# dwcoen1234/longfellow-zk

Hardware: AMD Instinct MI355X
Metric: FFT field-elems/s (batched FFT 2^20 x 1024 rows, Fp128) (higher is better)
Workload: dtype u128 (Fp128 Montgomery, 4 x u32 limbs); 1 GPU; batched FFT 2^20 points x 1024 rows per GPU, Fp128 fftb, in place in HBM; field=Fp128 p=2^128-2^108+1, rows_per_gpu=1024, n=1048576, parallelism=rows sharded x1

## Files before the change

longfellow-zk_amd/csrc/fft.hip:

```cpp
#include <string>
#include <type_traits>

#include "ctx.h"
#include "fp_tile_arith.h"

int lf_lch14_fft_bitsliced(lfgpu_ctx* c, int k, int inverse, size_t rows, unsigned l, u64 coset, void* d_B, size_t ld);

#define TILE_ELTS 8192u

struct TilePlan {
  const elt_t* src;
  elt_t* dst;
  long long src_row, dst_row;
  long long src_tile, dst_tile;
  long long sk, sc, dk, dc;
  u32 logT, logC, nbatch;
  u32 kfast_src, kfast_dst;
  u32 wlds;
};

__device__ __forceinline__ u32 bitrev(u32 x, u32 bits) { return bits ? (__brev(x) >> (32 - bits)) : 0; }

__device__ __forceinline__ u32 lds_slot(u32 k, u32 c, u32 logT, u32 logC) {
  u32 slot = (k << logC) + c;
// ... 102 lines not shown
      if (R == 3) fp_radix_round<O, 3, FFT_THREADS>(s, W, wsh, p.logT, p.logC, st, tid);
      else if (R == 2) fp_radix_round<O, 2, FFT_THREADS>(s, W, wsh, p.logT, p.logC, st, tid);
      else fp_radix_round<O, 1, FFT_THREADS>(s, W, wsh, p.logT, p.logC, st, tid);
    }
    __syncthreads();
    st += R;
  }
  for (u32 e = tid; e < T * C; e += FFT_THREADS) {
    u32 j, c;
    if (p.kfast_dst) { j = e & (T - 1); c = e >> p.logT; } else { c = e & (C - 1); j = e >> p.logC; }
    if (cbase + c >= p.nbatch) continue;
    elt_t v = ld16(&s[lds_slot(j, c, p.logT, p.logC)]);
    if (tw_lo) {
      const u32 col = cbase + c, ex = j * col;
      if (ex) {
        if (tw_hi) {
          elt_t t = ld16(&tw_lo[ex & 1023]);
          if (ex >> 10) t = O::mul_tw(t, ld16(&tw_hi[ex >> 10]));
          v = O::mul_tw(v, t);
        } else {
          v = O::mul_tw(v, ld16(&tw_lo[(size_t)j * p.nbatch + col]));
        }
      }
    }
    st16(dst + (long long)j * p.dk + (long long)c * p.dc, v);
  }
}

template <class O>
struct T4Ops : O {
  static __device__ __forceinline__ elt_t add_lazy(elt_t a, elt_t b) { return O::add(a, b); }
  static __device__ __forceinline__ elt_t canon(elt_t a) { return a; }
  static __device__ __forceinline__ elt_t mul_tw_sw(elt_t a, elt_t w) { return O::mul_tw(a, w); }
};
#if defined(__HIP_DEVICE_COMPILE__)
template <>
struct T4Ops<Fp128Ops> : Fp128Ops {
  static __device__ __forceinline__ elt_t add(elt_t a, elt_t b) { return fpt_add(a, b); }
  static __device__ __forceinline__ elt_t add_lazy(elt_t a, elt_t b) { return fpt_add_lazy(a, b); }
  static __device__ __forceinline__ elt_t canon(elt_t a) { return fpt_canon(a); }
  static __device__ __forceinline__ elt_t sub(elt_t a, elt_t b) { return fpt_sub(a, b); }
  static __device__ __forceinline__ elt_t mul_tw(elt_t a, elt_t w) { return fpt_mul(a, w); }
  static __device__ __forceinline__ elt_t mul_tw_sw(elt_t a, elt_t w) { return fpt_mul_sw(a, w); }
};
#endif

__device__ __forceinline__ u32 t4_slot(u32 p, u32 c, u32 p7) { return ((p << 2) | c) ^ p7; }
__device__ __forceinline__ u32 t4_wslot(u32 i) { return i ^ ((i >> 4) & 15u); }

enum : u32 { T4_CANON = 0, T4_LAZY = 1, T4_LAZY_OUT = 2 };
template <class O, u32 ST, u32 R, bool ROUND0, u32 LZ = T4_CANON>
__device__ __forceinline__ void t4_stages(elt_t* x, u32 j, const elt_t* wl, const elt_t* __restrict__ W, u32 wshift) {
#pragma unroll
  for (u32 t = 0; t < R; ++t) {
    const u32 half = 1u << t;
#pragma unroll
    for (u32 a = 0; a < (1u << R); ++a) {
      if (a & half) continue;
      const u32 jj = j + (a & (half - 1)) * (1u << ST), sh = 9 - ST - t;
      if (!ROUND0) x[a + half] = T4Ops<O>::mul_tw(x[a + half], ld16(&wl[t4_wslot(jj << sh)]));
      else if (a & (half - 1)) x[a + half] = T4Ops<O>::mul_tw(x[a + half], ld16(&W[(size_t)(jj << sh) << wshift]));
      const bool last = LZ == T4_LAZY_OUT && t == R - 1;
      const bool full = LZ == T4_CANON || last || (ROUND0 && ((t == 0 && a != 0) || (t == 1 && a == 4)));
      const elt_t u = last ? T4Ops<O>::canon(x[a]) : x[a], v = x[a + half];
      x[a] = full ? T4Ops<O>::add(u, v) : T4Ops<O>::add_lazy(u, v);
      x[a + half] = T4Ops<O>::sub(u, v);
    }
  }
}

template <class O, u32 LZ>
__device__ __forceinline__ void t4_round0(elt_t* s, const elt_t* y, u32 kb, u32 c, const elt_t* wl, const elt_t* __restrict__ W, u32 wshift) {
  elt_t x[8];
#pragma unroll
  for (u32 a = 0; a < 8; ++a) x[a] = y[((a & 1) << 2) | (a & 2) | (a >> 2)];
  t4_stages<O, 0, 3, true, LZ>(x, 0, wl, W, wshift);
  const u32 b = __brev(kb) >> 25, s0 = t4_slot(8 * b, c, b >> 4), s1 = t4_slot(8 * b + 1, c, b >> 4);
#pragma unroll
// ... 223 lines not shown
  fp_fft_tile_1024x4_tws_body<O, KFAST_SRC, true>(p, W, wshift, tw, row_fast);
}
template <class O, bool KFAST_SRC>
__global__ __launch_bounds__(512, 4) void fp_fft_tile_1024x4_tws_canon(TilePlan p, const elt_t* __restrict__ W, u32 wshift,
                                                                       const elt_t* __restrict__ tw, u32 row_fast) {
  fp_fft_tile_1024x4_tws_body<O, KFAST_SRC, false>(p, W, wshift, tw, row_fast);
}

__device__ __forceinline__ u32 t4w_swz(u32 p) { return (p >> 7) ^ ((p >> 4) & 12u); }
__device__ __forceinline__ u32 t4w_slot(u32 p, u32 c) { return ((p << 2) | c) ^ t4w_swz(p); }

template <u32 ST>
__device__ __forceinline__ u32 t4w_tw_index(u32 j, u32 m) {
  const u32 t = m < 1 ? 0 : m < 3 ? 1 : 2, k = m + 1 - (1u << t);
  return (j + (k << ST)) << (9 - ST - t);
}
enum : u32 { T4W_R0 = 0, T4W_R1 = 1, T4W_R1_J0 = 2 };
template <class O, u32 MODE>
__device__ __forceinline__ void t4w_stages(elt_t* x, const elt_t* w) {
#pragma unroll
  for (u32 t = 0; t < 3; ++t) {
    const u32 half = 1u << t;
#pragma unroll
    for (u32 a = 0; a < 8; ++a) {
      if (a & half) continue;
      const u32 k = a & (half - 1);
      const bool skip = MODE != T4W_R1 && k == 0, full = MODE == T4W_R0 && ((t == 0 && a != 0) || (t == 1 && a == 4));
      const elt_t u = x[a], v = !skip ? T4Ops<O>::mul_tw_sw(x[a + half], w[half - 1 + k]) : MODE == T4W_R1_J0 ? T4Ops<O>::canon(x[a + half]) : x[a + half];
      x[a] = full ? T4Ops<O>::add(u, v) : T4Ops<O>::add_lazy(u, v);
      x[a + half] = T4Ops<O>::sub(u, v);
    }
  }
}
template <class O>
__device__ __forceinline__ void t4w_round0(elt_t* s, const elt_t* y, u32 kb, u32 c, const elt_t* w) {
  elt_t x[8];
#pragma unroll
  for (u32 a = 0; a < 8; ++a) x[a] = y[((a & 1) << 2) | (a & 2) | (a >> 2)];
  t4w_stages<O, T4W_R0>(x, w);
  const u32 s0 = t4w_slot((__brev(kb) >> 25) << 3, c);
#pragma unroll
  for (u32 a = 0; a < 8; ++a) st16(&s[(s0 ^ (4 * (a & 3))) + 16 * (a >> 2)], x[a]);
}
template <class O, u32 MODE>
__device__ __forceinline__ void t4w_round1_wave(elt_t* s, u32 s0, const elt_t* w) {
  elt_t x[8];
#pragma unroll
  for (u32 a = 0; a < 8; ++a) x[a] = ld16(&s[s0 + 32 * a]);
  t4w_stages<O, MODE>(x, w);
#pragma unroll
  for (u32 a = 0; a < 8; ++a) st16(&s[s0 + 32 * a], x[a]);
}
template <class O>
__device__ __forceinline__ void t4w_round1(elt_t* s, u32 tid, u32 j, const elt_t* w) {
  const u32 c = tid & 3, h = (tid >> 2) & 15;
  const u32 s0 = t4w_slot(64 * h + j, c);
  if (j == 0) {
    asm volatile("; round 1, j = 0");
    t4w_round1_wave<O, T4W_R1_J0>(s, s0, w);
    asm volatile("; round 1, j = 0: stored");
  } else {
    asm volatile("; round 1, j > 0");
    t4w_round1_wave<O, T4W_R1>(s, s0, w);
    asm volatile("; round 1, j > 0: stored");
  }
}
template <class O>
__device__ __forceinline__ void t4w_round2(elt_t* s, u32 e, const elt_t* wl, const elt_t* __restrict__ W, u32 wshift) {
  const u32 c = e & 3, h = e >> 8, j = (e >> 2) & 63;
  const u32 s0 = t4w_slot(256 * h + j, c);
  elt_t x[4];
#pragma unroll
  for (u32 a = 0; a < 4; ++a) x[a] = ld16(&s[(s0 ^ t4w_swz(64 * a)) + 256 * a]);
  t4_stages<O, 6, 2, false, T4_LAZY>(x, j, wl, W, wshift);
#pragma unroll
  for (u32 a = 0; a < 4; ++a) st16(&s[(s0 ^ t4w_swz(64 * a)) + 256 * a], x[a]);
}
__device__ __forceinline__ void t4w_round3_load(elt_t* x, const elt_t* s, u32 e) {
  const u32 s0 = t4w_slot(e >> 2, e & 3);
#pragma unroll
  for (u32 a = 0; a < 4; ++a) x[a] = ld16(&s[(s0 ^ (2 * a)) + 1024 * a]);
}

template <class O, bool KFAST_SRC>
__global__ __launch_bounds__(512, 4) void fp_fft_tile_1024x4_tw2(TilePlan p, const elt_t* __restrict__ W, u32 wshift,
                                                                 const elt_t* __restrict__ tw, u32 row_fast) {
  extern __shared__ elt_t s[];
  elt_t* const wl = s + 4096;
  const u32 tid = threadIdx.x, j1 = __builtin_amdgcn_readfirstlane(tid >> 6);
  u32 bx, by;
  if (KFAST_SRC) {
    bx = row_fast ? blockIdx.y : blockIdx.x;
    by = row_fast ? blockIdx.x : blockIdx.y;
  } else {
    t4_xcd_order(p.nbatch >> 2, blockIdx.x, bx, by);
  }
  elt_t w0[7] = {}, w1[7];
  {
    const u32 c = KFAST_SRC ? tid >> 7 : tid & 3, kb = KFAST_SRC ? tid & 127 : tid >> 2;
    const elt_t* src = p.src + (long long)by * p.src_row + (long long)bx * p.src_tile;
    const u32 sk = (u32)p.sk, off = kb * sk + c * (u32)p.sc;
    elt_t y[8], t[8];
#pragma unroll
    for (u32 a = 0; a < 8; ++a) y[a] = ld16(src + (off + 128 * a * sk));
    if (KFAST_SRC) {
      const elt_t* twt = tw + ((size_t)bx << 12);
      const u32 toff = (c << 10) + kb;
#pragma unroll
      for (u32 a = 0; a < 8; ++a) t[a] = ld16(twt + (toff + 128 * a));
    }
    const elt_t wv = ld16(&W[(size_t)tid << wshift]);
#pragma unroll
    for (u32 m = 0; m < 7; ++m) {
      w1[m] = ld16(&W[(size_t)t4w_tw_index<3>(j1, m) << wshift]);
      if (m >= 4) w0[m] = ld16(&W[(size_t)t4w_tw_index<0>(0, m) << wshift]);
    }
#pragma unroll
    for (u32 m = 0; m < 7; ++m) {
      asm volatile("" : "+s"(w1[m].lo), "+s"(w1[m].hi));
      if (m >= 4) asm volatile("" : "+s"(w0[m].lo), "+s"(w0[m].hi));
    }
    w0[2] = w0[5];
    __builtin_amdgcn_sched_barrier(0);
    if (KFAST_SRC) {
#pragma unroll
      for (u32 a = 0; a < 8; ++a) y[a] = T4Ops<O>::mul_tw(y[a], t[a]);
    }
    t4w_round0<O>(s, y, kb, c, w0);
    st16(&wl[t4_wslot(tid)], wv);
  }
  __syncthreads();
  t4w_round1<O>(s, tid, j1, w1);
  __syncthreads();
#pragma unroll
  for (u32 g = 0; g < 2; ++g) t4w_round2<O>(s, tid + 512 * g, wl, W, wshift);
  __syncthreads();
  {
    elt_t* dst = p.dst + (long long)by * p.dst_row + (long long)bx * p.dst_tile;
    const u32 dk = (u32)p.dk, dc = (u32)p.dc;
#pragma unroll
    for (u32 g = 0; g < 2; ++g) {
      const u32 e = tid + 512 * g, c = e & 3, j = e >> 2;
      elt_t x[4];
      t4w_round3_load(x, s, e);
      t4_stages<O, 8, 2, false, KFAST_SRC ? T4_LAZY_OUT : T4_LAZY>(x, j, wl, W, wshift);
#pragma unroll
      for (u32 a = 0; a < 4; ++a) st16(dst + ((j + 256 * a) * dk + c * dc), x[a]);
    }
  }
}

struct LchTables {
  const elt_t* tbl;
  const elt_t* base;
  u32 nb;
  u32 off[16];
};

template <int FFT_THREADS>
__global__ __launch_bounds__(FFT_THREADS) void lch_fft_tile(TilePlan p, int inverse, LchTables t) {
  extern __shared__ elt_t s[];
  const u32 T = 1u << p.logT, C = 1u << p.logC, tid = threadIdx.x;
  const u32 cbase = blockIdx.x << p.logC;
  const elt_t* src = p.src + (long long)blockIdx.y * p.src_row + (long long)blockIdx.x * p.src_tile;
  elt_t* dst = p.dst + (long long)blockIdx.y * p.dst_row + (long long)blockIdx.x * p.dst_tile;

  for (u32 e = tid; e < T * C; e += FFT_THREADS) {
    u32 k, c;
    if (p.kfast_src) { k = e & (T - 1); c = e >> p.logT; } else { c = e & (C - 1); k = e >> p.logC; }
    elt_t v = elt_zero();
    if (cbase + c < p.nbatch) v = ld16(src + (long long)k * p.sk + (long long)c * p.sc);
    st16(&s[(k << p.logC) + c], v);
  }
  __syncthreads();
  for (u32 step = 0; step < p.logT; ++step) {
    const u32 ii = inverse ? step : (p.logT - 1 - step);
    const u32 sz = 1u << ii;
    for (u32 e = tid; e < (T >> 1) * C; e += FFT_THREADS) {
// ... 21 lines not shown
    __syncthreads();
  }
  for (u32 e = tid; e < T * C; e += FFT_THREADS) {
    u32 j, c;
    if (p.kfast_dst) { j = e & (T - 1); c = e >> p.logT; } else { c = e & (C - 1); j = e >> p.logC; }
    if (cbase + c >= p.nbatch) continue;
    st16(dst + (long long)j * p.dk + (long long)c * p.dc, ld16(&s[(j << p.logC) + c]));
  }
}

template <class O>
static int set_lds_limit_fp(lfgpu_ctx* c) {
  LF_HIP(c, hipFuncSetAttribute((const void*)fp_fft_tile<O, 1024, true>, hipFuncAttributeMaxDynamicSharedMemorySize, 160 * 1024));
  LF_HIP(c, hipFuncSetAttribute((const void*)fp_fft_tile<O, 1024, false>, hipFuncAttributeMaxDynamicSharedMemorySize, 160 * 1024));
  LF_HIP(c, hipFuncSetAttribute((const void*)fp_fft_tile<O, 512, true>, hipFuncAttributeMaxDynamicSharedMemorySize, 160 * 1024));
  LF_HIP(c, hipFuncSetAttribute((const void*)fp_fft_tile<O, 512, false>, hipFuncAttributeMaxDynamicSharedMemorySize, 160 * 1024));
  return LFGPU_OK;
}
static int set_lds_limit(lfgpu_ctx* c) {
  if (!(c->attr_done & 1u)) {
    if (const char* e = getenv("LFGPU_TILE_LOG")) {
      int v = atoi(e);
      if (v == 12 || v == 13) c->tile_log = v;
    }
    LF_TRY(set_lds_limit_fp<Fp128Ops>(c));
    const void* const t4[] = {(const void*)fp_fft_tile_1024x4<Fp128Ops, false, true>,
                              (const void*)fp_fft_tile_1024x4<Fp128Ops, true, false>,
                              (const void*)fp_fft_tile_1024x4_persist<Fp128Ops>,
                              (const void*)fp_fft_tile_1024x4_tws<Fp128Ops, false>,
                              (const void*)fp_fft_tile_1024x4_tws<Fp128Ops, true>,
                              (const void*)fp_fft_tile_1024x4_tws_canon<Fp128Ops, false>,
                              (const void*)fp_fft_tile_1024x4_tws_canon<Fp128Ops, true>,
                              (const void*)fp_fft_tile_1024x4_tw2<Fp128Ops, false>,
                              (const void*)fp_fft_tile_1024x4_tw2<Fp128Ops, true>};
    for (const void* k : t4) LF_HIP(c, hipFuncSetAttribute(k, hipFuncAttributeMaxDynamicSharedMemorySize, 160 * 1024));
    LF_TRY(set_lds_limit_fp<F64x2Ops<true>>(c));
    LF_TRY(set_lds_limit_fp<F64x2Ops<false>>(c));
    LF_HIP(c, hipFuncSetAttribute((const void*)lch_fft_tile<1024>, hipFuncAttributeMaxDynamicSharedMemorySize, TILE_ELTS * 16));
    LF_HIP(c, hipFuncSetAttribute((const void*)lch_fft_tile<512>, hipFuncAttributeMaxDynamicSharedMemorySize, TILE_ELTS * 16));
    c->attr_done |= 1u;
  }
  return LFGPU_OK;
}

static size_t fp_lds_bytes(TilePlan& p) {
  const size_t tile = ((size_t)16 << p.logT) << p.logC, tw = (size_t)8 << p.logT;
  p.wlds = tile + tw <= 160u * 1024u ? 1u : 0u;
  return p.wlds ? tile + tw : tile;
}
template <class O, class... Args>
static void launch_fp(lfgpu_ctx* c, dim3 grid, size_t lds, const TilePlan& p, Args... args) {
  if (c->tile_log == 13) {
    if (p.wlds) hipLaunchKernelGGL((fp_fft_tile<O, 1024, true>), grid, dim3(1024), lds, c->stream, p, args...);
    else hipLaunchKernelGGL((fp_fft_tile<O, 1024, false>), grid, dim3(1024), lds, c->stream, p, args...);
  } else {
    if (p.wlds) hipLaunchKernelGGL((fp_fft_tile<O, 512, true>), grid, dim3(512), lds, c->stream, p, args...);
    else hipLaunchKernelGGL((fp_fft_tile<O, 512, false>), grid, dim3(512), lds, c->stream, p, args...);
  }
}
struct FpSwitches {
  bool tile1024;
  int persist;
  int twside;
  bool other_plan;
  bool lazy;
  bool r1wave;
  bool two_level;
  bool row_fast;
};
static const FpSwitches& fp_switches() {
  static const FpSwitches sw = [] {
    const auto num = [](const char* name, int dflt) { return getenv(name) ? atoi(getenv(name)) : dflt; };
    FpSwitches w;
    w.tile1024 = num("LFGPU_FP_TILE1024", 1) != 0;
    w.persist = num("LFGPU_FP_PERSIST", 1);
    w.twside = num("LFGPU_FP_TWSIDE", 1);
    w.other_plan = getenv("LFGPU_FP_PERSIST") || getenv("LFGPU_FP_TILE1024");
    w.lazy = num("LFGPU_FP_LAZY", 1) != 0;
    w.r1wave = num("LFGPU_FP_R1WAVE", 1) != 0;
    w.two_level = num("LFGPU_FP_TW", 0) == 2;
    w.row_fast = num("LFGPU_FP_ROWFAST", 1) != 0;
    return w;
  }();
  return sw;
}
static bool tile_1024x4_fits(const TilePlan& p, bool kfast_src, bool offsets32) {
  if (p.logT != 10 || p.logC != 2 || !p.wlds || p.kfast_src != (kfast_src ? 1u : 0u) || p.kfast_dst != 0 || (p.nbatch & 3) != 0) return false;
  return !offsets32 || (p.sk >= 0 && p.sc >= 0 && p.dk >= 0 && p.dc >= 0 && (u64)p.sk * 1024 + (u64)p.sc * 4 <= 0xffffffffu &&
                        (u64)p.dk * 1024 + (u64)p.dc * 4 <= 0xffffffffu);
}
template <class O>
static bool launch_tile_1024x4_persist(lfgpu_ctx* c, u32 rows, size_t lds, const TilePlan& p, const elt_t* W, u32 wshift, const elt_t* tw) {
  const int mode = fp_switches().persist;
  const u32 ncb = p.nbatch >> 2;
  u32 parts = rows;
  if (mode <= 0 || !tile_1024x4_fits(p, false, true)) return false;
  if (mode >= 2) {
    static const int per_cu = [lds] {
      int n = 0;
      if (hipOccupancyMaxActiveBlocksPerMultiprocessor(&n, (const void*)fp_fft_tile_1024x4_persist<O>, 512, lds) != hipSuccess)
        n = 0;
      return n < 1 ? 1 : n;
    }();
    const u32 fill = (u32)per_cu * (u32)c->num_cu;
    parts = fill / ncb;
    if (parts < 1) parts = 1;
    if (parts > rows) parts = rows;
  }
  if ((u64)ncb * parts > 0x7fffffffu) return false;
  const dim3 grid(ncb * parts);
  hipLaunchKernelGGL((fp_fft_tile_1024x4_persist<O>), grid, dim3(512), lds, c->stream, p, W, wshift, tw, rows, parts);
  return true;
}
template <class O, bool KFAST_SRC, bool TW>
static bool launch_tile_1024x4(lfgpu_ctx* c, dim3 grid, size_t lds, const TilePlan& p, const elt_t* W, u32 wshift, const elt_t* tw,
                               u32 row_fast) {
  if constexpr (std::is_same<O, Fp128Ops>::value) {
    if (fp_switches().tile1024 && c->tile_log == 12 && tile_1024x4_fits(p, KFAST_SRC, false)) {
      if constexpr (!KFAST_SRC && TW)
        if (launch_tile_1024x4_persist<O>(c, row_fast ? grid.x : grid.y, lds, p, W, wshift, tw)) return true;
      hipLaunchKernelGGL((fp_fft_tile_1024x4<O, KFAST_SRC, TW>), grid, dim3(512), lds, c->stream, p, W, wshift, tw, row_fast);
      return true;
    }
  }
  return false;
}
template <class O>
static int fp_twside_mode(const lfgpu_ctx* c, u32 logn1, size_t rows, bool two_level) {
  const int mode = fp_switches().other_plan ? 0 : fp_switches().twside;
  if (!std::is_same<O, Fp128Ops>::value || two_level || c->tile_log != 12 || logn1 != 10 || rows > (0x7fffffffu >> 8)) return 0;
  return mode < 0 ? 0 : mode;
}
template <class O, bool KFAST_SRC>
static bool launch_tile_1024x4_tws(lfgpu_ctx* c, u32 rows, size_t lds, const TilePlan& p, const elt_t* W, u32 wshift, const elt_t* tw,
                                   u32 row_fast) {
  if constexpr (std::is_same<O, Fp128Ops>::value) {
    const u32 ncb = p.nbatch >> 2;
    if (!tile_1024x4_fits(p, KFAST_SRC, true) || (u64)ncb * rows > 0x7fffffffu) return false;
    if (KFAST_SRC && (p.sk != 1 || p.sc != 1024 || p.src_tile != 4096)) return false;
    if (KFAST_SRC && (row_fast ? ncb : rows) > 65535) row_fast = !row_fast;
    const dim3 grid = !KFAST_SRC ? dim3(ncb * rows) : row_fast ? dim3(rows, ncb) : dim3(ncb, rows);
    if (!fp_switches().lazy) hipLaunchKernelGGL((fp_fft_tile_1024x4_tws_canon<O, KFAST_SRC>), grid, dim3(512), lds, c->stream, p, W, wshift, tw, row_fast);
    else if (fp_switches().r1wave) hipLaunchKernelGGL((fp_fft_tile_1024x4_tw2<O, KFAST_SRC>), grid, dim3(512), lds, c->stream, p, W, wshift, tw, row_fast);
    else hipLaunchKernelGGL((fp_fft_tile_1024x4_tws<O, KFAST_SRC>), grid, dim3(512), lds, c->stream, p, W, wshift, tw, row_fast);
    return true;
  }
  return false;
}
template <class... Args>
static void launch_lch(lfgpu_ctx* c, dim3 grid, size_t lds, Args... args) {
  if (c->tile_log == 13)
    hipLaunchKernelGGL(lch_fft_tile<1024>, grid, dim3(1024), lds, c->stream, args...);
  else
    hipLaunchKernelGGL(lch_fft_tile<512>, grid, dim3(512), lds, c->stream, args...);
}

template <class O>
static elt_t fp_reroot(elt_t w, u64 n, u64 r) {
  while (r < n) {
    w = O::hmul(w, w);
    r += r;
  }
  return w;
}

static std::string keyf(const char* fmt, ...) {
  char buf[256];
  va_list ap;
  va_start(ap, fmt);
  vsnprintf(buf, sizeof(buf), fmt, ap);
  va_end(ap);
  return std::string(buf);
}

static TilePlan plan_single(const lfgpu_ctx* c, void* A, size_t rows, u32 logn, size_t ld) {
// ... 359 lines not shown
```

longfellow-zk_amd/csrc/fp_tile_arith.h:

```cpp
#pragma once
#include "fields.h"

#if defined(__HIP_DEVICE_COMPILE__)
__device__ __forceinline__ elt_t fpt_add(elt_t a, elt_t b) {
  FP_W(a, a0, a1, a2, a3);
  FP_W(b, b0, b1, b2, b3);
  u32 s0, s1, s2, s3, d0, d1, d2, d3;
  u64 c;
  asm("v_add_co_u32 %0, vcc, %9, %13\n\t"
      "s_nop 1\n\t"
      "v_addc_co_u32 %1, vcc, %10, %14, vcc\n\t"
      "s_nop 1\n\t"
      "v_addc_co_u32 %2, vcc, %11, %15, vcc\n\t"
      "s_nop 1\n\t"
      "v_addc_co_u32 %3, %8, %12, %16, vcc\n\t"
      "v_subrev_co_u32 %4, vcc, 1, %0\n\t"
      "s_nop 1\n\t"
      "v_subbrev_co_u32 %5, vcc, 0, %1, vcc\n\t"
      "s_nop 1\n\t"
      "v_subbrev_co_u32 %6, vcc, 0, %2, vcc\n\t"
      "s_nop 1\n\t"
      "v_subb_co_u32 %7, vcc, %3, %17, vcc\n\t"
      "s_nop 1\n\t"
      "s_andn2_b64 vcc, vcc, %8\n\t"
// ... 139 lines not shown
        "s_nop 1\n\t"
        "v_subb_co_u32 %2, vcc, %15, %6, vcc\n\t"
        "s_nop 1\n\t"
        "v_subb_co_u32 %3, %10, %16, %7, vcc\n\t"
        "v_alignbit_b32 %4, %5, %4, 20\n\t"
        "v_alignbit_b32 %5, %6, %5, 20\n\t"
        "v_alignbit_b32 %6, %7, %6, 20\n\t"
        "v_lshrrev_b32 %7, 20, %7\n\t"
        "v_addc_co_u32 %0, vcc, %0, %4, %9\n\t"
        "s_nop 1\n\t"
        "v_addc_co_u32 %1, vcc, %1, %5, vcc\n\t"
        "s_nop 1\n\t"
        "v_addc_co_u32 %2, vcc, %2, %6, vcc\n\t"
        "s_nop 1\n\t"
        "v_addc_co_u32 %3, %9, %3, %7, vcc\n\t"
        "s_nop 1\n\t"
        "s_andn2_b64 %9, %10, %9\n\t"
        "v_cndmask_b32 %8, 0, %12, %9\n\t"
        "v_addc_co_u32 %0, vcc, 0, %0, %9\n\t"
        "s_nop 1\n\t"
        "v_addc_co_u32 %1, vcc, 0, %1, vcc\n\t"
        "s_nop 1\n\t"
        "v_addc_co_u32 %2, vcc, 0, %2, vcc\n\t"
        "s_nop 1\n\t"
        "v_addc_co_u32 %3, vcc, %8, %3, vcc"
        : "=&v"(d0), "=&v"(d1), "=&v"(d2), "=&v"(d3), "+v"(t0), "+v"(t1), "+v"(t2), "+v"(t3), "=&v"(e3), "=&s"(cy), "=&s"(b)
        : "v"(k), "v"(0xfffff000u), "v"(t4), "v"(t5), "v"(t6), "v"(t7)
        : "vcc", "scc");
  }
  return FP_PACK(d0, d1, d2, d3);
}
__device__ __forceinline__ elt_t fpt_mul(elt_t a, elt_t b) { return fpt_mul_t<false>(a, b); }
__device__ __forceinline__ elt_t fpt_mul_sw(elt_t a, elt_t b) { return fpt_mul_t<true>(a, b); }
#else
LF_HD elt_t fpt_add(elt_t a, elt_t b) { return fp_add_c(a, b); }
LF_HD elt_t fpt_sub(elt_t a, elt_t b) { return fp_sub_c(a, b); }
LF_HD elt_t fpt_canon(elt_t a) { return fp_canon128(a); }
LF_HD elt_t fpt_add_lazy(elt_t a, elt_t b) {
  const u64 lo = a.lo + b.lo, c0 = lo < a.lo, h0 = a.hi + b.hi, hi = h0 + c0;
  if (!((h0 < a.hi) | (hi < c0))) return elt_t{lo, hi};
  return elt_t{lo - FP_P_LO, hi - FP_P_HI - (lo < FP_P_LO)};
}
LF_HD elt_t fpt_mul(elt_t a, elt_t b) { return fp_mul_c(fp_canon128(a), b); }
LF_HD elt_t fpt_mul_sw(elt_t a, elt_t b) { return fpt_mul(a, b); }
#endif
```

Baseline: 48.89 billion field-elems/s.

## Interleave paired Fp128 multiplies and butterflies in inline asm for ILP

```diff
diff --git a/longfellow-zk_amd/csrc/fft.hip b/longfellow-zk_amd/csrc/fft.hip
--- a/longfellow-zk_amd/csrc/fft.hip
+++ b/longfellow-zk_amd/csrc/fft.hip
@@ -158,6 +158,14 @@
   static __device__ __forceinline__ elt_t add_lazy(elt_t a, elt_t b) { return O::add(a, b); }
   static __device__ __forceinline__ elt_t canon(elt_t a) { return a; }
   static __device__ __forceinline__ elt_t mul_tw_sw(elt_t a, elt_t w) { return O::mul_tw(a, w); }
+  static __device__ __forceinline__ void mul2_tw(elt_t& a, elt_t w, elt_t& b, elt_t v) { a = O::mul_tw(a, w), b = O::mul_tw(b, v); }
+  static __device__ __forceinline__ void mul2_tw_sw(elt_t& a, elt_t w, elt_t& b, elt_t v) { mul2_tw(a, w, b, v); }
+  static __device__ __forceinline__ void canon2(elt_t&, elt_t&) {}
+  static __device__ __forceinline__ void bfly_lazy(elt_t& x, elt_t& y) {
+    const elt_t u = x, t = y;
+    x = O::add(u, t), y = O::sub(u, t);
+  }
+  static __device__ __forceinline__ void bfly2_lazy(elt_t& xp, elt_t& yp, elt_t& xq, elt_t& yq) { bfly_lazy(xp, yp), bfly_lazy(xq, yq); }
 };
 #if defined(__HIP_DEVICE_COMPILE__)
 template <>
@@ -168,8 +176,21 @@
   static __device__ __forceinline__ elt_t sub(elt_t a, elt_t b) { return fpt_sub(a, b); }
   static __device__ __forceinline__ elt_t mul_tw(elt_t a, elt_t w) { return fpt_mul(a, w); }
   static __device__ __forceinline__ elt_t mul_tw_sw(elt_t a, elt_t w) { return fpt_mul_sw(a, w); }
+  static __device__ __forceinline__ void mul2_tw(elt_t& a, elt_t w, elt_t& b, elt_t v) { fpt_mul2(a, w, b, v); }
+  static __device__ __forceinline__ void mul2_tw_sw(elt_t& a, elt_t w, elt_t& b, elt_t v) { fpt_mul2_sw(a, w, b, v); }
+  static __device__ __forceinline__ void canon2(elt_t& a, elt_t& b) { fpt_canon2(a, b); }
+  static __device__ __forceinline__ void bfly_lazy(elt_t& x, elt_t& y) { fpt_bfly_lazy(x, y); }
+  static __device__ __forceinline__ void bfly2_lazy(elt_t& xp, elt_t& yp, elt_t& xq, elt_t& yq) { fpt_bfly2_lazy(xp, yp, xq, yq); }
 };
 #endif
+template <class O>
+struct T4Ilp : O {};
+template <class O>
+struct T4IsIlp : std::false_type {};
+template <class O>
+struct T4IsIlp<T4Ilp<O>> : std::true_type {};
+template <class O>
+struct T4Ops<T4Ilp<O>> : T4Ops<O> {};
 
 __device__ __forceinline__ u32 t4_slot(u32 p, u32 c, u32 p7) { return ((p << 2) | c) ^ p7; }
 __device__ __forceinline__ u32 t4_wslot(u32 i) { return i ^ ((i >> 4) & 15u); }
@@ -459,12 +480,79 @@
     }
   }
 }
+struct T4iStage {
+  u32 np, prod[4], nc, can[4], nl, lazy[4], nf, full[4];
+};
+template <u32 MODE>
+constexpr T4iStage t4i_plan(u32 t) {
+  T4iStage s{};
+  const u32 half = 1u << t;
+  for (u32 a = 0; a < 8; ++a) {
+    if (a & half) continue;
+    const bool skip = MODE != T4W_R1 && (a & (half - 1)) == 0, full = MODE == T4W_R0 && ((t == 0 && a != 0) || (t == 1 && a == 4));
+    if (!skip) s.prod[s.np++] = a;
+    else if (MODE == T4W_R1_J0) s.can[s.nc++] = a;
+    if (full) s.full[s.nf++] = a;
+    else s.lazy[s.nl++] = a;
+  }
+  return s;
+}
+template <class O, u32 MODE, u32 T>
+__device__ __forceinline__ void t4i_stage(elt_t* x, const elt_t* w) {
+  constexpr T4iStage S = t4i_plan<MODE>(T);
+  constexpr u32 half = 1u << T, first = half - 1;
+#pragma unroll
+  for (u32 i = 0; i + 1 < S.np; i += 2) {
+    const u32 a = S.prod[i], b = S.prod[i + 1];
+    T4Ops<O>::mul2_tw_sw(x[a + half], w[first + (a & first)], x[b + half], w[first + (b & first)]);
+  }
+  if constexpr (S.np & 1) x[S.prod[S.np - 1] + half] = T4Ops<O>::mul_tw_sw(x[S.prod[S.np - 1] + half], w[first + (S.prod[S.np - 1] & first)]);
+#pragma unroll
+  for (u32 i = 0; i + 1 < S.nc; i += 2) T4Ops<O>::canon2(x[S.can[i] + half], x[S.can[i + 1] + half]);
+  if constexpr (S.nc & 1) x[S.can[S.nc - 1] + half] = T4Ops<O>::canon(x[S.can[S.nc - 1] + half]);
+#pragma unroll
+  for (u32 i = 0; i < S.nf; ++i) {
+    const u32 a = S.full[i];
+    const elt_t u = x[a], v = x[a + half];
+    x[a] = T4Ops<O>::add(u, v);
+    x[a + half] = T4Ops<O>::sub(u, v);
+  }
+#pragma unroll
+  for (u32 i = 0; i + 1 < S.nl; i += 2) T4Ops<O>::bfly2_lazy(x[S.lazy[i]], x[S.lazy[i] + half], x[S.lazy[i + 1]], x[S.lazy[i + 1] + half]);
+  if constexpr (S.nl & 1) T4Ops<O>::bfly_lazy(x[S.lazy[S.nl - 1]], x[S.lazy[S.nl - 1] + half]);
+}
+template <class O, u32 MODE>
+__device__ __forceinline__ void t4i_stages(elt_t* x, const elt_t* w) {
+  t4i_stage<O, MODE, 0>(x, w);
+  t4i_stage<O, MODE, 1>(x, w);
+  t4i_stage<O, MODE, 2>(x, w);
+}
+template <class O, u32 ST, u32 LZ>
+__device__ __forceinline__ void t4i_stages4(elt_t* x, u32 j, const elt_t* wl) {
+#pragma unroll
+  for (u32 t = 0; t < 2; ++t) {
+    const u32 half = 1u << t, a = 0, b = 2 >> t, sh = 9 - ST - t;
+    T4Ops<O>::mul2_tw(x[a + half], ld16(&wl[t4_wslot(j << sh)]), x[b + half], ld16(&wl[t4_wslot((j + (b & (half - 1)) * (1u << ST)) << sh)]));
+    if (LZ == T4_LAZY_OUT && t == 1) {
+      T4Ops<O>::canon2(x[a], x[b]);
+#pragma unroll
+      for (u32 i = 0; i < 2; ++i) {
+        const elt_t u = x[i], v = x[i + half];
+        x[i] = T4Ops<O>::add(u, v);
+        x[i + half] = T4Ops<O>::sub(u, v);
+      }
+    } else {
+      T4Ops<O>::bfly2_lazy(x[a], x[a + half], x[b], x[b + half]);
+    }
+  }
+}
 template <class O>
 __device__ __forceinline__ void t4w_round0(elt_t* s, const elt_t* y, u32 kb, u32 c, const elt_t* w) {
   elt_t x[8];
 #pragma unroll
   for (u32 a = 0; a < 8; ++a) x[a] = y[((a & 1) << 2) | (a & 2) | (a >> 2)];
-  t4w_stages<O, T4W_R0>(x, w);
+  if constexpr (T4IsIlp<O>::value) t4i_stages<O, T4W_R0>(x, w);
+  else t4w_stages<O, T4W_R0>(x, w);
   const u32 s0 = t4w_slot((__brev(kb) >> 25) << 3, c);
 #pragma unroll
   for (u32 a = 0; a < 8; ++a) st16(&s[(s0 ^ (4 * (a & 3))) + 16 * (a >> 2)], x[a]);
@@ -474,7 +562,8 @@
   elt_t x[8];
 #pragma unroll
   for (u32 a = 0; a < 8; ++a) x[a] = ld16(&s[s0 + 32 * a]);
-  t4w_stages<O, MODE>(x, w);
+  if constexpr (T4IsIlp<O>::value) t4i_stages<O, MODE>(x, w);
+  else t4w_stages<O, MODE>(x, w);
 #pragma unroll
   for (u32 a = 0; a < 8; ++a) st16(&s[s0 + 32 * a], x[a]);
 }
@@ -499,7 +588,8 @@
   elt_t x[4];
 #pragma unroll
   for (u32 a = 0; a < 4; ++a) x[a] = ld16(&s[(s0 ^ t4w_swz(64 * a)) + 256 * a]);
-  t4_stages<O, 6, 2, false, T4_LAZY>(x, j, wl, W, wshift);
+  if constexpr (T4IsIlp<O>::value) t4i_stages4<O, 6, T4_LAZY>(x, j, wl);
+  else t4_stages<O, 6, 2, false, T4_LAZY>(x, j, wl, W, wshift);
 #pragma unroll
   for (u32 a = 0; a < 4; ++a) st16(&s[(s0 ^ t4w_swz(64 * a)) + 256 * a], x[a]);
 }
@@ -550,8 +640,13 @@
     w0[2] = w0[5];
     __builtin_amdgcn_sched_barrier(0);
     if (KFAST_SRC) {
-#pragma unroll
-      for (u32 a = 0; a < 8; ++a) y[a] = T4Ops<O>::mul_tw(y[a], t[a]);
+      if constexpr (T4IsIlp<O>::value) {
+#pragma unroll
+        for (u32 a = 0; a < 8; a += 2) T4Ops<O>::mul2_tw(y[a], t[a], y[a + 1], t[a + 1]);
+      } else {
+#pragma unroll
+        for (u32 a = 0; a < 8; ++a) y[a] = T4Ops<O>::mul_tw(y[a], t[a]);
+      }
     }
     t4w_round0<O>(s, y, kb, c, w0);
     st16(&wl[t4_wslot(tid)], wv);
@@ -570,7 +665,8 @@
       const u32 e = tid + 512 * g, c = e & 3, j = e >> 2;
       elt_t x[4];
       t4w_round3_load(x, s, e);
-      t4_stages<O, 8, 2, false, KFAST_SRC ? T4_LAZY_OUT : T4_LAZY>(x, j, wl, W, wshift);
+      if constexpr (T4IsIlp<O>::value) t4i_stages4<O, 8, KFAST_SRC ? T4_LAZY_OUT : T4_LAZY>(x, j, wl);
+      else t4_stages<O, 8, 2, false, KFAST_SRC ? T4_LAZY_OUT : T4_LAZY>(x, j, wl, W, wshift);
 #pragma unroll
       for (u32 a = 0; a < 4; ++a) st16(dst + ((j + 256 * a) * dk + c * dc), x[a]);
     }
@@ -658,7 +754,9 @@
                               (const void*)fp_fft_tile_1024x4_tws_canon<Fp128Ops, false>,
                               (const void*)fp_fft_tile_1024x4_tws_canon<Fp128Ops, true>,
                               (const void*)fp_fft_tile_1024x4_tw2<Fp128Ops, false>,
-                              (const void*)fp_fft_tile_1024x4_tw2<Fp128Ops, true>};
+                              (const void*)fp_fft_tile_1024x4_tw2<Fp128Ops, true>,
+                              (const void*)fp_fft_tile_1024x4_tw2<T4Ilp<Fp128Ops>, false>,
+                              (const void*)fp_fft_tile_1024x4_tw2<T4Ilp<Fp128Ops>, true>};
     for (const void* k : t4) LF_HIP(c, hipFuncSetAttribute(k, hipFuncAttributeMaxDynamicSharedMemorySize, 160 * 1024));
     LF_TRY(set_lds_limit_fp<F64x2Ops<true>>(c));
     LF_TRY(set_lds_limit_fp<F64x2Ops<false>>(c));
@@ -691,6 +789,7 @@
   bool other_plan;
   bool lazy;
   bool r1wave;
+  bool ilp;
   bool two_level;
   bool row_fast;
 };
@@ -704,6 +803,7 @@
     w.other_plan = getenv("LFGPU_FP_PERSIST") || getenv("LFGPU_FP_TILE1024");
     w.lazy = num("LFGPU_FP_LAZY", 1) != 0;
     w.r1wave = num("LFGPU_FP_R1WAVE", 1) != 0;
+    w.ilp = num("LFGPU_FP_ILP", 1) != 0;
     w.two_level = num("LFGPU_FP_TW", 0) == 2;
     w.row_fast = num("LFGPU_FP_ROWFAST", 1) != 0;
     return w;
@@ -767,6 +867,7 @@
     if (KFAST_SRC && (row_fast ? ncb : rows) > 65535) row_fast = !row_fast;
     const dim3 grid = !KFAST_SRC ? dim3(ncb * rows) : row_fast ? dim3(rows, ncb) : dim3(ncb, rows);
     if (!fp_switches().lazy) hipLaunchKernelGGL((fp_fft_tile_1024x4_tws_canon<O, KFAST_SRC>), grid, dim3(512), lds, c->stream, p, W, wshift, tw, row_fast);
+    else if (fp_switches().r1wave && fp_switches().ilp) hipLaunchKernelGGL((fp_fft_tile_1024x4_tw2<T4Ilp<O>, KFAST_SRC>), grid, dim3(512), lds, c->stream, p, W, wshift, tw, row_fast);
     else if (fp_switches().r1wave) hipLaunchKernelGGL((fp_fft_tile_1024x4_tw2<O, KFAST_SRC>), grid, dim3(512), lds, c->stream, p, W, wshift, tw, row_fast);
     else hipLaunchKernelGGL((fp_fft_tile_1024x4_tws<O, KFAST_SRC>), grid, dim3(512), lds, c->stream, p, W, wshift, tw, row_fast);
     return true;
diff --git a/longfellow-zk_amd/csrc/fp_tile_arith.h b/longfellow-zk_amd/csrc/fp_tile_arith.h
--- a/longfellow-zk_amd/csrc/fp_tile_arith.h
+++ b/longfellow-zk_amd/csrc/fp_tile_arith.h
@@ -195,6 +195,297 @@
 }
 __device__ __forceinline__ elt_t fpt_mul(elt_t a, elt_t b) { return fpt_mul_t<false>(a, b); }
 __device__ __forceinline__ elt_t fpt_mul_sw(elt_t a, elt_t b) { return fpt_mul_t<true>(a, b); }
+
+
+__device__ __forceinline__ void fpt_bfly2_lazy(elt_t& xp, elt_t& yp, elt_t& xq, elt_t& yq) {
+  FP_W(xp, up0, up1, up2, up3);
+  FP_W(yp, tp0, tp1, tp2, tp3);
+  FP_W(xq, uq0, uq1, uq2, uq3);
+  FP_W(yq, tq0, tq1, tq2, tq3);
+  u32 dp0, dp1, dp2, dp3, dq0, dq1, dq2, dq3, eap, esp, eaq, esq;
+  u64 c1, c2, c3;
+  asm("v_add_co_u32 %[dp0], vcc, %[up0], %[tp0]\n\t"
+      "v_sub_co_u32 %[tp0], %[c1], %[up0], %[tp0]\n\t"
+      "v_add_co_u32 %[dq0], %[c2], %[uq0], %[tq0]\n\t"
+      "v_sub_co_u32 %[tq0], %[c3], %[uq0], %[tq0]\n\t"
+      "v_addc_co_u32 %[dp1], vcc, %[up1], %[tp1], vcc\n\t"
+      "v_subb_co_u32 %[tp1], %[c1], %[up1], %[tp1], %[c1]\n\t"
+      "v_addc_co_u32 %[dq1], %[c2], %[uq1], %[tq1], %[c2]\n\t"
+      "v_subb_co_u32 %[tq1], %[c3], %[uq1], %[tq1], %[c3]\n\t"
+      "v_addc_co_u32 %[dp2], vcc, %[up2], %[tp2], vcc\n\t"
+      "v_subb_co_u32 %[tp2], %[c1], %[up2], %[tp2], %[c1]\n\t"
+      "v_addc_co_u32 %[dq2], %[c2], %[uq2], %[tq2], %[c2]\n\t"
+      "v_subb_co_u32 %[tq2], %[c3], %[uq2], %[tq2], %[c3]\n\t"
+      "v_addc_co_u32 %[dp3], vcc, %[up3], %[tp3], vcc\n\t"
+      "v_subb_co_u32 %[tp3], %[c1], %[up3], %[tp3], %[c1]\n\t"
+      "v_addc_co_u32 %[dq3], %[c2], %[uq3], %[tq3], %[c2]\n\t"
+      "v_subb_co_u32 %[tq3], %[c3], %[uq3], %[tq3], %[c3]\n\t"
+      "v_cndmask_b32 %[eap], 0, %[k], vcc\n\t"
+      "v_cndmask_b32 %[esp], 0, %[k], %[c1]\n\t"
+      "v_cndmask_b32 %[eaq], 0, %[k], %[c2]\n\t"
+      "v_cndmask_b32 %[esq], 0, %[k], %[c3]\n\t"
+      "v_subbrev_co_u32 %[dp0], vcc, 0, %[dp0], vcc\n\t"
+      "v_addc_co_u32 %[tp0], %[c1], 0, %[tp0], %[c1]\n\t"
+      "v_subbrev_co_u32 %[dq0], %[c2], 0, %[dq0], %[c2]\n\t"
+      "v_addc_co_u32 %[tq0], %[c3], 0, %[tq0], %[c3]\n\t"
+      "v_subbrev_co_u32 %[dp1], vcc, 0, %[dp1], vcc\n\t"
+      "v_addc_co_u32 %[tp1], %[c1], 0, %[tp1], %[c1]\n\t"
+      "v_subbrev_co_u32 %[dq1], %[c2], 0, %[dq1], %[c2]\n\t"
+      "v_addc_co_u32 %[tq1], %[c3], 0, %[tq1], %[c3]\n\t"
+      "v_subbrev_co_u32 %[dp2], vcc, 0, %[dp2], vcc\n\t"
+      "v_addc_co_u32 %[tp2], %[c1], 0, %[tp2], %[c1]\n\t"
+      "v_subbrev_co_u32 %[dq2], %[c2], 0, %[dq2], %[c2]\n\t"
+      "v_addc_co_u32 %[tq2], %[c3], 0, %[tq2], %[c3]\n\t"
+      "v_subb_co_u32 %[dp3], vcc, %[dp3], %[eap], vcc\n\t"
+      "v_addc_co_u32 %[tp3], %[c1], %[esp], %[tp3], %[c1]\n\t"
+      "v_subb_co_u32 %[dq3], %[c2], %[dq3], %[eaq], %[c2]\n\t"
+      "v_addc_co_u32 %[tq3], %[c3], %[esq], %[tq3], %[c3]"
+      : [dp0] "=&v"(dp0), [dp1] "=&v"(dp1), [dp2] "=&v"(dp2), [dp3] "=&v"(dp3), [dq0] "=&v"(dq0), [dq1] "=&v"(dq1), [dq2] "=&v"(dq2),
+        [dq3] "=&v"(dq3), [tp0] "+v"(tp0), [tp1] "+v"(tp1), [tp2] "+v"(tp2), [tp3] "+v"(tp3), [tq0] "+v"(tq0), [tq1] "+v"(tq1),
+        [tq2] "+v"(tq2), [tq3] "+v"(tq3), [eap] "=&v"(eap), [esp] "=&v"(esp), [eaq] "=&v"(eaq), [esq] "=&v"(esq), [c1] "=&s"(c1),
+        [c2] "=&s"(c2), [c3] "=&s"(c3)
+      : [up0] "v"(up0), [up1] "v"(up1), [up2] "v"(up2), [up3] "v"(up3), [uq0] "v"(uq0), [uq1] "v"(uq1), [uq2] "v"(uq2), [uq3] "v"(uq3),
+        [k] "v"(0xfffff000u)
+      : "vcc");
+  xp = FP_PACK(dp0, dp1, dp2, dp3);
+  yp = FP_PACK(tp0, tp1, tp2, tp3);
+  xq = FP_PACK(dq0, dq1, dq2, dq3);
+  yq = FP_PACK(tq0, tq1, tq2, tq3);
+}
+
+__device__ __forceinline__ void fpt_bfly_lazy(elt_t& x, elt_t& y) {
+  FP_W(x, u0, u1, u2, u3);
+  FP_W(y, t0, t1, t2, t3);
+  u32 d0, d1, d2, d3, y0, y1, y2, y3, ea, es;
+  u64 c1;
+  asm("v_add_co_u32 %[d0], vcc, %[u0], %[t0]\n\t"
+      "v_sub_co_u32 %[y0], %[c1], %[u0], %[t0]\n\t"
+      "s_nop 0\n\t"
+      "v_addc_co_u32 %[d1], vcc, %[u1], %[t1], vcc\n\t"
+      "v_subb_co_u32 %[y1], %[c1], %[u1], %[t1], %[c1]\n\t"
+      "s_nop 0\n\t"
+      "v_addc_co_u32 %[d2], vcc, %[u2], %[t2], vcc\n\t"
+      "v_subb_co_u32 %[y2], %[c1], %[u2], %[t2], %[c1]\n\t"
+      "s_nop 0\n\t"
+      "v_addc_co_u32 %[d3], vcc, %[u3], %[t3], vcc\n\t"
+      "v_subb_co_u32 %[y3], %[c1], %[u3], %[t3], %[c1]\n\t"
+      "s_nop 0\n\t"
+      "v_cndmask_b32 %[ea], 0, %[k], vcc\n\t"
+      "v_cndmask_b32 %[es], 0, %[k], %[c1]\n\t"
+      "v_subbrev_co_u32 %[d0], vcc, 0, %[d0], vcc\n\t"
+      "v_addc_co_u32 %[y0], %[c1], 0, %[y0], %[c1]\n\t"
+      "s_nop 0\n\t"
+      "v_subbrev_co_u32 %[d1], vcc, 0, %[d1], vcc\n\t"
+      "v_addc_co_u32 %[y1], %[c1], 0, %[y1], %[c1]\n\t"
+      "s_nop 0\n\t"
+      "v_subbrev_co_u32 %[d2], vcc, 0, %[d2], vcc\n\t"
+      "v_addc_co_u32 %[y2], %[c1], 0, %[y2], %[c1]\n\t"
+      "s_nop 0\n\t"
+      "v_subb_co_u32 %[d3], vcc, %[d3], %[ea], vcc\n\t"
+      "v_addc_co_u32 %[y3], %[c1], %[es], %[y3], %[c1]"
+      : [d0] "=&v"(d0), [d1] "=&v"(d1), [d2] "=&v"(d2), [d3] "=&v"(d3), [y0] "=&v"(y0), [y1] "=&v"(y1), [y2] "=&v"(y2), [y3] "=&v"(y3),
+        [ea] "=&v"(ea), [es] "=&v"(es), [c1] "=&s"(c1)
+      : [u0] "v"(u0), [u1] "v"(u1), [u2] "v"(u2), [u3] "v"(u3), [t0] "v"(t0), [t1] "v"(t1), [t2] "v"(t2), [t3] "v"(t3), [k] "v"(0xfffff000u)
+      : "vcc");
+  x = FP_PACK(d0, d1, d2, d3);
+  y = FP_PACK(y0, y1, y2, y3);
+}
+
+__device__ __forceinline__ void fpt_canon2(elt_t& p, elt_t& q) {
+  FP_W(p, a0, a1, a2, a3);
+  FP_W(q, b0, b1, b2, b3);
+  u32 d0, d1, d2, d3, e0, e1, e2, e3;
+  u64 c1;
+  asm("v_subrev_co_u32 %[d0], vcc, 1, %[a0]\n\t"
+      "v_subrev_co_u32 %[e0], %[c1], 1, %[b0]\n\t"
+      "s_nop 0\n\t"
+      "v_subbrev_co_u32 %[d1], vcc, 0, %[a1], vcc\n\t"
+      "v_subbrev_co_u32 %[e1], %[c1], 0, %[b1], %[c1]\n\t"
+      "s_nop 0\n\t"
+      "v_subbrev_co_u32 %[d2], vcc, 0, %[a2], vcc\n\t"
+      "v_subbrev_co_u32 %[e2], %[c1], 0, %[b2], %[c1]\n\t"
+      "s_nop 0\n\t"
+      "v_subb_co_u32 %[d3], vcc, %[a3], %[k], vcc\n\t"
+      "v_subb_co_u32 %[e3], %[c1], %[b3], %[k], %[c1]\n\t"
+      "s_nop 0\n\t"
+      "v_cndmask_b32 %[d0], %[d0], %[a0], vcc\n\t"
+      "v_cndmask_b32 %[d1], %[d1], %[a1], vcc\n\t"
+      "v_cndmask_b32 %[d2], %[d2], %[a2], vcc\n\t"
+      "v_cndmask_b32 %[d3], %[d3], %[a3], vcc\n\t"
+      "v_cndmask_b32 %[e0], %[e0], %[b0], %[c1]\n\t"
+      "v_cndmask_b32 %[e1], %[e1], %[b1], %[c1]\n\t"
+      "v_cndmask_b32 %[e2], %[e2], %[b2], %[c1]\n\t"
+      "v_cndmask_b32 %[e3], %[e3], %[b3], %[c1]"
+      : [d0] "=&v"(d0), [d1] "=&v"(d1), [d2] "=&v"(d2), [d3] "=&v"(d3), [e0] "=&v"(e0), [e1] "=&v"(e1), [e2] "=&v"(e2), [e3] "=&v"(e3),
+        [c1] "=&s"(c1)
+      : [a0] "v"(a0), [a1] "v"(a1), [a2] "v"(a2), [a3] "v"(a3), [b0] "v"(b0), [b1] "v"(b1), [b2] "v"(b2), [b3] "v"(b3), [k] "v"(0xfffff000u)
+      : "vcc");
+  p = FP_PACK(d0, d1, d2, d3);
+  q = FP_PACK(e0, e1, e2, e3);
+}
+
+#define FPT_M2 "v_mad_u64_u32 "
+#define FPT_C2 "v_addc_co_u32 "
+#define FPT_COLUMNS2(C)                                                                                                          \
+  asm(FPT_M2 "%[pacc], vcc, %[pa0], %[pb0], 0\n\t"                                                                                \
+      FPT_M2 "%[qacc], vcc, %[qa0], %[qb0], 0"                                                                                    \
+      : [pacc] "=&v"(pacc0), [qacc] "=&v"(qacc0)                                                                                  \
+      : [pa0] "v"(pa0), [pb0] C(pb0), [qa0] "v"(qa0), [qb0] C(qb0)                                                                \
+      : "vcc");                                                                                                                   \
+  pt0 = (u32)pacc0;                                                                                                               \
+  qt0 = (u32)qacc0;                                                                                                               \
+  asm("v_lshrrev_b64 %[qin], 32, %[qacc0]\n\t"                                                                                    \
+      FPT_M2 "%[pacc], vcc, %[pa0], %[pb1], %[pin]\n\t"                                                                           \
+      FPT_M2 "%[qacc], vcc, %[qa0], %[qb1], %[qin]\n\t"                                                                           \
+      FPT_M2 "%[pacc], %[s1], %[pa1], %[pb0], %[pacc]\n\t"                                                                        \
+      FPT_M2 "%[qacc], %[s2], %[qa1], %[qb0], %[qacc]\n\t"                                                                        \
+      "s_nop 0\n\t"                                                                                                               \
+      FPT_C2 "%[pov], vcc, 0, 0, %[s1]\n\t"                                                                                       \
+      FPT_C2 "%[qov], vcc, 0, 0, %[s2]"                                                                                           \
+      : [pacc] "=&v"(pacc), [qacc] "=&v"(qacc), [pov] "=&v"(pov), [qov] "=&v"(qov), [s1] "=&s"(s1), [s2] "=&s"(s2),               \
+        [qin] "=&v"(qin)                                                                                                          \
+      : [pa0] "v"(pa0), [pa1] "v"(pa1), [pb0] C(pb0), [pb1] C(pb1), [qa0] "v"(qa0), [qa1] "v"(qa1), [qb0] C(qb0), [qb1] C(qb1),   \
+        [pin] "v"(pacc0 >> 32), [qacc0] "v"(qacc0)                                                                                \
+      : "vcc");                                                                                                                   \
+  FPT_COL(pt1, pacc, pov);                                                                                                        \
+  FPT_COL(qt1, qacc, qov);                                                                                                        \
+  FPT_COLUMN2_3(C, 0, 2, 1, 1, 2, 0);                                                                                             \
+  FPT_COL(pt2, pacc, pov);                                                                                                        \
+  FPT_COL(qt2, qacc, qov);                                                                                                        \
+  asm(FPT_M2 "%[pacc], vcc, %[pa0], %[pb3], %[pacc]\n\t"                                                                          \
+      FPT_M2 "%[qacc], vcc, %[qa0], %[qb3], %[qacc]\n\t"                                                                          \
+      FPT_M2 "%[pacc], %[s1], %[pa1], %[pb2], %[pacc]\n\t"                                                                        \
+      FPT_M2 "%[qacc], %[s2], %[qa1], %[qb2], %[qacc]\n\t"                                                                        \
+      FPT_M2 "%[pacc], %[s3], %[pa2], %[pb1], %[pacc]\n\t"                                                                        \
+      FPT_M2 "%[qacc], %[s4], %[qa2], %[qb1], %[qacc]\n\t"                                                                        \
+      FPT_M2 "%[pacc], %[s5], %[pa3], %[pb0], %[pacc]\n\t"                                                                        \
+      FPT_M2 "%[qacc], %[s6], %[qa3], %[qb0], %[qacc]\n\t"                                                                        \
+      FPT_C2 "%[pov], vcc, 0, 0, %[s1]\n\t"                                                                                       \
+      FPT_C2 "%[qov], vcc, 0, 0, %[s2]\n\t"                                                                                       \
+      FPT_C2 "%[pov], vcc, 0, %[pov], %[s3]\n\t"                                                                                  \
+      FPT_C2 "%[qov], vcc, 0, %[qov], %[s4]\n\t"                                                                                  \
+      FPT_C2 "%[pov], vcc, 0, %[pov], %[s5]\n\t"                                                                                  \
+      FPT_C2 "%[qov], vcc, 0, %[qov], %[s6]"                                                                                      \
+      : [pacc] "+v"(pacc), [qacc] "+v"(qacc), [pov] "=&v"(pov), [qov] "=&v"(qov), [s1] "=&s"(s1), [s2] "=&s"(s2), [s3] "=&s"(s3), \
+        [s4] "=&s"(s4), [s5] "=&s"(s5), [s6] "=&s"(s6)                                                                            \
+      : [pa0] "v"(pa0), [pa1] "v"(pa1), [pa2] "v"(pa2), [pa3] "v"(pa3), [pb0] C(pb0), [pb1] C(pb1), [pb2] C(pb2), [pb3] C(pb3),   \
+        [qa0] "v"(qa0), [qa1] "v"(qa1), [qa2] "v"(qa2), [qa3] "v"(qa3), [qb0] C(qb0), [qb1] C(qb1), [qb2] C(qb2), [qb3] C(qb3)    \
+      : "vcc");                                                                                                                   \
+  FPT_COL(pt3, pacc, pov);                                                                                                        \
+  FPT_COL(qt3, qacc, qov);                                                                                                        \
+  FPT_COLUMN2_3(C, 1, 3, 2, 2, 3, 1);                                                                                             \
+  FPT_COL(pt4, pacc, pov);                                                                                                        \
+  FPT_COL(qt4, qacc, qov);                                                                                                        \
+  asm(FPT_M2 "%[pacc], vcc, %[pa2], %[pb3], %[pacc]\n\t"                                                                          \
+      FPT_M2 "%[qacc], vcc, %[qa2], %[qb3], %[qacc]\n\t"                                                                          \
+      FPT_M2 "%[pacc], %[s1], %[pa3], %[pb2], %[pacc]\n\t"                                                                        \
+      FPT_M2 "%[qacc], %[s2], %[qa3], %[qb2], %[qacc]\n\t"                                                                        \
+      "s_nop 0\n\t"                                                                                                               \
+      FPT_C2 "%[pov], vcc, 0, 0, %[s1]\n\t"                                                                                       \
+      FPT_C2 "%[qov], vcc, 0, 0, %[s2]"                                                                                           \
+      : [pacc] "+v"(pacc), [qacc] "+v"(qacc), [pov] "=&v"(pov), [qov] "=&v"(qov), [s1] "=&s"(s1), [s2] "=&s"(s2)                  \
+      : [pa2] "v"(pa2), [pa3] "v"(pa3), [pb2] C(pb2), [pb3] C(pb3), [qa2] "v"(qa2), [qa3] "v"(qa3), [qb2] C(qb2), [qb3] C(qb3)    \
+      : "vcc");                                                                                                                   \
+  FPT_COL(pt5, pacc, pov);                                                                                                        \
+  FPT_COL(qt5, qacc, qov);                                                                                                        \
+  asm(FPT_M2 "%[pacc], vcc, %[pa3], %[pb3], %[pacc]\n\t"                                                                          \
+      FPT_M2 "%[qacc], vcc, %[qa3], %[qb3], %[qacc]"                                                                              \
+      : [pacc] "+v"(pacc), [qacc] "+v"(qacc)                                                                                      \
+      : [pa3] "v"(pa3), [pb3] C(pb3), [qa3] "v"(qa3), [qb3] C(qb3)                                                                \
+      : "vcc");                                                                                                                   \
+  pt6 = (u32)pacc;                                                                                                                \
+  pt7 = (u32)(pacc >> 32);                                                                                                        \
+  qt6 = (u32)qacc;                                                                                                                \
+  qt7 = (u32)(qacc >> 32)
+#define FPT_COLUMN2_3(C, i, j, k, l, m, n)                                                                                        \
+  asm(FPT_M2 "%[pacc], vcc, %[pi], %[pj], %[pacc]\n\t"                                                                            \
+      FPT_M2 "%[qacc], vcc, %[qi], %[qj], %[qacc]\n\t"                                                                            \
+      FPT_M2 "%[pacc], %[s1], %[pk], %[pl], %[pacc]\n\t"                                                                          \
+      FPT_M2 "%[qacc], %[s2], %[qk], %[ql], %[qacc]\n\t"                                                                          \
+      FPT_M2 "%[pacc], %[s3], %[pm], %[pn], %[pacc]\n\t"                                                                          \
+      FPT_M2 "%[qacc], %[s4], %[qm], %[qn], %[qacc]\n\t"                                                                          \
+      FPT_C2 "%[pov], vcc, 0, 0, %[s1]\n\t"                                                                                       \
+      FPT_C2 "%[qov], vcc, 0, 0, %[s2]\n\t"                                                                                       \
+      FPT_C2 "%[pov], vcc, 0, %[pov], %[s3]\n\t"                                                                                  \
+      FPT_C2 "%[qov], vcc, 0, %[qov], %[s4]"                                                                                      \
+      : [pacc] "+v"(pacc), [qacc] "+v"(qacc), [pov] "=&v"(pov), [qov] "=&v"(qov), [s1] "=&s"(s1), [s2] "=&s"(s2), [s3] "=&s"(s3), \
+        [s4] "=&s"(s4)                                                                                                            \
+      : [pi] "v"(pa##i), [pk] "v"(pa##k), [pm] "v"(pa##m), [pj] C(pb##j), [pl] C(pb##l), [pn] C(pb##n), [qi] "v"(qa##i),          \
+        [qk] "v"(qa##k), [qm] "v"(qa##m), [qj] C(qb##j), [ql] C(qb##l), [qn] C(qb##n)                                             \
+      : "vcc")
+
+template <bool SW>
+__device__ __forceinline__ void fpt_mul2_t(elt_t& pa, elt_t pw, elt_t& qa, elt_t qw) {
+  FP_W(pa, pa0, pa1, pa2, pa3);
+  FP_W(pw, pb0, pb1, pb2, pb3);
+  FP_W(qa, qa0, qa1, qa2, qa3);
+  FP_W(qw, qb0, qb1, qb2, qb3);
+  u32 pt0, pt1, pt2, pt3, pt4, pt5, pt6, pt7, pov, qt0, qt1, qt2, qt3, qt4, qt5, qt6, qt7, qov;
+  u64 pacc0, pacc, qacc0, qacc, qin, s1, s2, s3, s4, s5, s6;
+  if constexpr (SW) {
+    FPT_COLUMNS2("s");
+  } else {
+    FPT_COLUMNS2("v");
+  }
+  const u32 pk = pt0 << 12, qk = qt0 << 12;
+  u32 pd0, pd1, pd2, pd3, qd0, qd1, qd2, qd3, pe, qe;
+  u64 pcy, pb, qcy, qb, qs;
+  asm("v_add_co_u32 %[pt3], %[pcy], %[pt3], %[pk]\n\t"
+      "v_add_co_u32 %[qt3], %[qcy], %[qt3], %[qk]\n\t"
+      "v_sub_co_u32 %[pd0], vcc, %[pt4], %[pt0]\n\t"
+      "v_sub_co_u32 %[qd0], %[qs], %[qt4], %[qt0]\n\t"
+      "v_alignbit_b32 %[pt0], %[pt1], %[pt0], 20\n\t"
+      "v_alignbit_b32 %[qt0], %[qt1], %[qt0], 20\n\t"
+      "v_subb_co_u32 %[pd1], vcc, %[pt5], %[pt1], vcc\n\t"
+      "v_subb_co_u32 %[qd1], %[qs], %[qt5], %[qt1], %[qs]\n\t"
+      "v_alignbit_b32 %[pt1], %[pt2], %[pt1], 20\n\t"
+      "v_alignbit_b32 %[qt1], %[qt2], %[qt1], 20\n\t"
+      "v_subb_co_u32 %[pd2], vcc, %[pt6], %[pt2], vcc\n\t"
+      "v_subb_co_u32 %[qd2], %[qs], %[qt6], %[qt2], %[qs]\n\t"
+      "v_alignbit_b32 %[pt2], %[pt3], %[pt2], 20\n\t"
+      "v_alignbit_b32 %[qt2], %[qt3], %[qt2], 20\n\t"
+      "v_subb_co_u32 %[pd3], %[pb], %[pt7], %[pt3], vcc\n\t"
+      "v_subb_co_u32 %[qd3], %[qb], %[qt7], %[qt3], %[qs]\n\t"
+      "v_lshrrev_b32 %[pt3], 20, %[pt3]\n\t"
+      "v_lshrrev_b32 %[qt3], 20, %[qt3]\n\t"
+      "v_addc_co_u32 %[pd0], vcc, %[pd0], %[pt0], %[pcy]\n\t"
+      "v_addc_co_u32 %[qd0], %[qs], %[qd0], %[qt0], %[qcy]\n\t"
+      "s_nop 0\n\t"
+      "v_addc_co_u32 %[pd1], vcc, %[pd1], %[pt1], vcc\n\t"
+      "v_addc_co_u32 %[qd1], %[qs], %[qd1], %[qt1], %[qs]\n\t"
+      "s_nop 0\n\t"
+      "v_addc_co_u32 %[pd2], vcc, %[pd2], %[pt2], vcc\n\t"
+      "v_addc_co_u32 %[qd2], %[qs], %[qd2], %[qt2], %[qs]\n\t"
+      "s_nop 0\n\t"
+      "v_addc_co_u32 %[pd3], %[pcy], %[pd3], %[pt3], vcc\n\t"
+      "v_addc_co_u32 %[qd3], %[qcy], %[qd3], %[qt3], %[qs]\n\t"
+      "s_nop 0\n\t"
+      "s_andn2_b64 %[pcy], %[pb], %[pcy]\n\t"
+      "s_andn2_b64 %[qcy], %[qb], %[qcy]\n\t"
+      "v_addc_co_u32 %[pd0], vcc, 0, %[pd0], %[pcy]\n\t"
+      "v_addc_co_u32 %[qd0], %[qs], 0, %[qd0], %[qcy]\n\t"
+      "v_cndmask_b32 %[pe], 0, %[k], %[pcy]\n\t"
+      "v_cndmask_b32 %[qe], 0, %[k], %[qcy]\n\t"
+      "v_addc_co_u32 %[pd1], vcc, 0, %[pd1], vcc\n\t"
+      "v_addc_co_u32 %[qd1], %[qs], 0, %[qd1], %[qs]\n\t"
+      "s_nop 0\n\t"
+      "v_addc_co_u32 %[pd2], vcc, 0, %[pd2], vcc\n\t"
+      "v_addc_co_u32 %[qd2], %[qs], 0, %[qd2], %[qs]\n\t"
+      "s_nop 0\n\t"
+      "v_addc_co_u32 %[pd3], vcc, %[pe], %[pd3], vcc\n\t"
+      "v_addc_co_u32 %[qd3], %[qs], %[qe], %[qd3], %[qs]"
+      : [pd0] "=&v"(pd0), [pd1] "=&v"(pd1), [pd2] "=&v"(pd2), [pd3] "=&v"(pd3), [qd0] "=&v"(qd0), [qd1] "=&v"(qd1), [qd2] "=&v"(qd2),
+        [qd3] "=&v"(qd3), [pt0] "+v"(pt0), [pt1] "+v"(pt1), [pt2] "+v"(pt2), [pt3] "+v"(pt3), [qt0] "+v"(qt0), [qt1] "+v"(qt1),
+        [qt2] "+v"(qt2), [qt3] "+v"(qt3), [pe] "=&v"(pe), [qe] "=&v"(qe), [pcy] "=&s"(pcy), [pb] "=&s"(pb), [qcy] "=&s"(qcy),
+        [qb] "=&s"(qb), [qs] "=&s"(qs)
+      : [pk] "v"(pk), [qk] "v"(qk), [k] "v"(0xfffff000u), [pt4] "v"(pt4), [pt5] "v"(pt5), [pt6] "v"(pt6), [pt7] "v"(pt7), [qt4] "v"(qt4),
+        [qt5] "v"(qt5), [qt6] "v"(qt6), [qt7] "v"(qt7)
+      : "vcc", "scc");
+  pa = FP_PACK(pd0, pd1, pd2, pd3);
+  qa = FP_PACK(qd0, qd1, qd2, qd3);
+}
+__device__ __forceinline__ void fpt_mul2(elt_t& pa, elt_t pw, elt_t& qa, elt_t qw) { fpt_mul2_t<false>(pa, pw, qa, qw); }
+__device__ __forceinline__ void fpt_mul2_sw(elt_t& pa, elt_t pw, elt_t& qa, elt_t qw) { fpt_mul2_t<true>(pa, pw, qa, qw); }
 #else
 LF_HD elt_t fpt_add(elt_t a, elt_t b) { return fp_add_c(a, b); }
 LF_HD elt_t fpt_sub(elt_t a, elt_t b) { return fp_sub_c(a, b); }
@@ -206,4 +497,22 @@
 }
 LF_HD elt_t fpt_mul(elt_t a, elt_t b) { return fp_mul_c(fp_canon128(a), b); }
 LF_HD elt_t fpt_mul_sw(elt_t a, elt_t b) { return fpt_mul(a, b); }
+LF_HD void fpt_bfly_lazy(elt_t& x, elt_t& y) {
+  const elt_t u = x, t = y;
+  x = fpt_add_lazy(u, t);
+  y = fpt_sub(u, t);
+}
+LF_HD void fpt_bfly2_lazy(elt_t& xp, elt_t& yp, elt_t& xq, elt_t& yq) {
+  fpt_bfly_lazy(xp, yp);
+  fpt_bfly_lazy(xq, yq);
+}
+LF_HD void fpt_canon2(elt_t& p, elt_t& q) {
+  p = fpt_canon(p);
+  q = fpt_canon(q);
+}
+LF_HD void fpt_mul2(elt_t& pa, elt_t pw, elt_t& qa, elt_t qw) {
+  pa = fpt_mul(pa, pw);
+  qa = fpt_mul(qa, qw);
+}
+LF_HD void fpt_mul2_sw(elt_t& pa, elt_t pw, elt_t& qa, elt_t qw) { fpt_mul2(pa, pw, qa, qw); }
 #endif
```

Result: faster. 50.26 billion field-elems/s (median of 6 runs) (+2.8%).
